# saiprasadbarke/robustmvd

Measured on AMD Instinct MI355X. Metric: depth-maps/sec at 768x1152x4srcx256planes; warp+aggregate HBM GB/s vs roofline, higher is better.
Workload: dtype f32; 1 GPU; mvsnet (Path B) forward 768x1152, 4 source views, 256 planes, batch 1 per step (BASELINE.json configs[2]); the regulariser's two layers with 32 input channels (conv0, conv4): every fp32 operand as two range-scaled fp16 terms on fp16 MFMA, fp32 accumulation (at least as close to a float64 convolution as the fp32 matrix instruction over 1e-42..1e30: tests/test_hip_f16.py), the other nine layers and ; parallelism=1 independent replica(s), frames round-robin, no collectives

## Files before the change

### robustmvd_amd/csrc/warp_variance_tile.hip

```cpp
#include "mvd_common.h"
#include <type_traits>
#include "warp_variance_common.h"

namespace mvd {

typedef unsigned short u16x2 __attribute__((ext_vector_type(2)));

__device__ __forceinline__ unsigned pk_min_u16(unsigned a, unsigned b) {
    return __builtin_bit_cast(unsigned, __builtin_elementwise_min(__builtin_bit_cast(u16x2, a), __builtin_bit_cast(u16x2, b)));
}
__device__ __forceinline__ unsigned pk_max_u16(unsigned a, unsigned b) {
    return __builtin_bit_cast(unsigned, __builtin_elementwise_max(__builtin_bit_cast(u16x2, a), __builtin_bit_cast(u16x2, b)));
}
template <int K>
__device__ __forceinline__ unsigned row_shr(unsigned v) {
    return (unsigned)__builtin_amdgcn_update_dpp((int)v, (int)v, 0x110 + K, 0xf, 0xf, false);
}

typedef float f32x2 __attribute__((ext_vector_type(2)));
struct Sums { f32x2 a1[2], a2[2]; };
__device__ __forceinline__ void tap_pairs(const u32x4& t, f32x2& lo, f32x2& hi) {
    lo = f32x2{__uint_as_float(t.x), __uint_as_float(t.y)};
    hi = f32x2{__uint_as_float(t.z), __uint_as_float(t.w)};
}
__device__ __forceinline__ void tap_pairs(const u32x2& t, f32x2& lo, f32x2& hi) {
    const f16x2 l = as_h2(t.x), h = as_h2(t.y);
    lo = f32x2{(float)l.x, (float)l.y};
    hi = f32x2{(float)h.x, (float)h.y};
}
template <class TAP>
__device__ __forceinline__ void accumulate_cell_pk(Sums& s, const float4 w, const TAP (&t)[4]) {
    const float wk[4] = {w.x, w.y, w.z, w.w};
    f32x2 lo = {0.0f, 0.0f}, hi = {0.0f, 0.0f};
#pragma unroll
    for (int k = 0; k < 4; ++k) {
        f32x2 tl, th;
        tap_pairs(t[k], tl, th);
        const f32x2 ws = {wk[k], wk[k]};
        lo = __builtin_elementwise_fma(tl, ws, lo);
        hi = __builtin_elementwise_fma(th, ws, hi);
    }
    s.a1[0] += lo; s.a1[1] += hi;
    s.a2[0] = __builtin_elementwise_fma(lo, lo, s.a2[0]);
    s.a2[1] = __builtin_elementwise_fma(hi, hi, s.a2[1]);
}

__device__ __forceinline__ void lds_dma_b128(u32x4 rsrc, unsigned voff, unsigned lds_dst) {
    asm volatile("s_mov_b32 m0, %2\n\ts_nop 0\n\tbuffer_load_dwordx4 %0, %1, 0 offen lds" : : "v"(voff), "s"(rsrc), "s"(lds_dst) : "memory");
}

#ifndef MVD_K3T_KO
#define MVD_K3T_KO 0
#endif

struct UnitRec {
    unsigned boxmin;
    unsigned extent;
    unsigned pitch;
    unsigned npix;
    unsigned base;
    unsigned skip;
    float inv_nc;
    unsigned pad;
};
struct ViewRec {
    float M[12];
    unsigned base_lo, base_hi;
    unsigned pad[2];
};

template <int TW, int WINPIX, bool F16, bool EXACT, int MINW, int SETS>
__global__ void __launch_bounds__(256, MINW) warp_variance_tile_kernel(WarpParams p, int nch) {
    constexpr int P = 8, NPX = 32;
    constexpr unsigned PIXB = F16 ? 64 : 128;
    constexpr unsigned QB = F16 ? 8 : 16;
    constexpr unsigned WINB = WINPIX * PIXB;
    constexpr int PPP = 1024 / PIXB;
    constexpr int LPX = PIXB / 16;
    constexpr int NPIECE = WINPIX / PPP;
    constexpr unsigned TABW0 = 2 * WINB, TABO0 = TABW0 + 2 * 4096, PROBE0 = TABO0 + 2 * 1024, FAIL0 = PROBE0 + 512, VIEW0 = FAIL0 + 128;
    using TAP = typename std::conditional<F16, u32x2, u32x4>::type;
    extern __shared__ __attribute__((aligned(16))) char lds[];

    const int tid = threadIdx.x;
    const int wv = __builtin_amdgcn_readfirstlane(tid >> 6);
    const int h = p.h, w = p.w, D = p.D, V = p.V;
    const unsigned DEP0 = VIEW0 + (unsigned)V * sizeof(ViewRec), UNIT0 = DEP0 + (unsigned)nch * 32;

    const int xcd = blockIdx.x & 7;
    int j = blockIdx.x >> 3;
    const int dchunks = (D + P - 1) / P;
    const int dgroups = (dchunks + nch - 1) / nch;
    const int dg = j % dgroups; j /= dgroups;
    const int tile_in = j % p.tiles_per_xcd;
    const int b = j / p.tiles_per_xcd;
    const int tile = xcd * p.tiles_per_xcd + tile_in;
    if (tile >= p.tiles_x * p.tiles_y) return;
    const int tyi = tile / p.tiles_x;
    const int x0 = (tile - tyi * p.tiles_x) * TW, y0 = tyi * (NPX / TW);
    const int nchunks = (dchunks - dg + dgroups - 1) / dgroups;
    auto chunk_of = [&](int jc) { return dg + jc * dgroups; };

    const int W2 = w + 3;
    const unsigned rowb = (unsigned)W2 * PIXB;
    const unsigned img_bytes = (unsigned)(h + 3) * rowb;

    auto opaque_tid = [&]() { int t = tid; asm volatile("" : "+v"(t)); return t; };
    auto blend_pixel = [&](int t, int& bx, int& by) {
        const int px = t >> 3;
        bx = min(x0 + px % TW, w - 1);
        by = min(y0 + px / TW, h - 1);
    };

    float4 key;
    {
        int bx, by;
        blend_pixel(tid, bx, by);
        const char* kp = reinterpret_cast<const char*>(p.key) + (size_t)b * img_bytes + (unsigned)(by + 1) * rowb +
                         (unsigned)(bx + 1) * PIXB + (unsigned)(tid & 7) * QB;
        if constexpr (F16) {
            const u32x2 kh = *reinterpret_cast<const u32x2*>(kp);
            const f16x2 lo = as_h2(kh.x), hi = as_h2(kh.y);
            key = make_float4((float)lo.x, (float)lo.y, (float)hi.x, (float)hi.y);
        } else {
            key = *reinterpret_cast<const float4*>(kp);
        }
    }
    const float inv_nv = 1.0f / (float)(V + 1);
    const size_t plane_bytes = (size_t)h * w * PIXB;

    auto src_rsrc = [&](int v) {
        return __builtin_amdgcn_make_buffer_rsrc(const_cast<char*>(reinterpret_cast<const char*>(p.src.p[v]) + (size_t)b * img_bytes),
                                                 0, (int)img_bytes, 0x00020000);
    };

    const float sx = __int_as_float(__builtin_amdgcn_readfirstlane(__float_as_int((float)w / (float)(w - 1))));
    const float sy = __int_as_float(__builtin_amdgcn_readfirstlane(__float_as_int((float)h / (float)(h - 1))));
    auto position = [&](const float (&M)[12], float fx, float fy, float depth, float& ix, float& iy) -> float {
        float Z;
        if constexpr (EXACT) {
            const float half_w = (float)(w - 1) / 2.0f, half_h = (float)(h - 1) / 2.0f;
            const float gx = fx * depth, gy = fy * depth;
            const float X = ((M[0] * gx + M[1] * gy) + M[2] * depth) + M[3];
            const float Y = ((M[4] * gx + M[5] * gy) + M[6] * depth) + M[7];
            Z = ((M[8] * gx + M[9] * gy) + M[10] * depth) + M[11];
            ix = unnormalize_coord((X / Z) / half_w - 1.0f, (float)w);
            iy = unnormalize_coord((Y / Z) / half_h - 1.0f, (float)h);
        } else {
            const float ax = fmaf(M[0], fx, fmaf(M[1], fy, M[2]));
            const float ay = fmaf(M[4], fx, fmaf(M[5], fy, M[6]));
            const float az = fmaf(M[8], fx, fmaf(M[9], fy, M[10]));
            const float X = fmaf(ax, depth, M[3]), Y = fmaf(ay, depth, M[7]);
            Z = fmaf(az, depth, M[11]);
            const float rz = __builtin_amdgcn_rcpf(Z);
            ix = fmaf(X * rz, sx, -0.5f);
            iy = fmaf(Y * rz, sy, -0.5f);
        }
        ix = __builtin_amdgcn_fmed3f(ix, -1.0f, (float)w);
        iy = __builtin_amdgcn_fmed3f(iy, -1.0f, (float)h);
        return Z;
    };

    unsigned lds_chunks;
    {
        const int pv = tid >> 3, co = tid & 7;
        const float cfx = (float)((co & 1) ? min(x0 + TW - 1, w - 1) : x0);
        const float cfy = (float)((co & 2) ? min(y0 + NPX / TW - 1, h - 1) : y0);
        float M[12];
        {
            const float* Mg = p.M + ((size_t)min(pv, V - 1) * p.B + b) * 12;
#pragma unroll
            for (int k = 0; k < 12; ++k) M[k] = Mg[k];
        }
        if (co == 0 && pv < V) {
            ViewRec* vr = reinterpret_cast<ViewRec*>(lds + VIEW0) + pv;
#pragma unroll
            for (int k = 0; k < 12; ++k) vr->M[k] = M[k];
            const unsigned long long sb = (unsigned long long)(reinterpret_cast<const char*>(p.src.p[pv]) + (size_t)b * img_bytes);
            vr->base_lo = (unsigned)sb; vr->base_hi = (unsigned)(sb >> 32);
        }
        if (tid < 32) *reinterpret_cast<unsigned*>(lds + FAIL0 + tid * 4) = 0u;
        const float* dg_ = p.depth + (size_t)b * D;
        for (int e = tid; e < nchunks * P; e += 256) *reinterpret_cast<float*>(lds + DEP0 + e * 4) = dg_[min(chunk_of(e / P) * P + e % P, D - 1)];
        __syncthreads();
        for (int jc = 0; jc < nchunks; ++jc) {
            const float depth = *reinterpret_cast<const float*>(lds + DEP0 + (jc * P + ((co & 4) ? P - 1 : 0)) * 4);
            float ix, iy;
            const float Z = position(M, cfx, cfy, depth, ix, iy);
            const unsigned cell = ((unsigned)((int)floorf(iy) + 1) << 16) | (unsigned)((int)floorf(ix) + 1);
            const bool ok = Z > 0.0f;
            unsigned mn = ok ? cell : 0u, mx = ok ? cell : 0xffffffffu;
            mn = pk_min_u16(mn, row_shr<1>(mn)); mx = pk_max_u16(mx, row_shr<1>(mx));
            mn = pk_min_u16(mn, row_shr<2>(mn)); mx = pk_max_u16(mx, row_shr<2>(mx));
            mn = pk_min_u16(mn, row_shr<4>(mn)); mx = pk_max_u16(mx, row_shr<4>(mx));
            const int xmin = max((int)(mn & 0xffffu) - 1, 0), ymin = max((int)(mn >> 16) - 1, 0);
            const int xmax = min((int)(mx & 0xffffu) + 1, w + 1), ymax = min((int)(mx >> 16) + 1, h + 1);
            const int nc = xmax - xmin + 2, nr = ymax - ymin + 2;
            const bool mine = (co == 7) && (pv < V);
            if (mine) {
                UnitRec r;
                r.boxmin = (unsigned)xmin | ((unsigned)ymin << 16);
                r.extent = (unsigned)(xmax - xmin) | ((unsigned)(ymax - ymin) << 16);
                r.pitch = (unsigned)nc * PIXB;
                r.npix = (unsigned)(nc * nr);
                r.base = (unsigned)(ymin * W2 + xmin) * PIXB;
                r.skip = rowb - (unsigned)nc * PIXB;
                r.inv_nc = 1.0f / (float)nc;
                r.pad = 0;
                *(reinterpret_cast<UnitRec*>(lds + UNIT0) + jc * V + pv) = r;
            }
            const bool any_bad = __builtin_amdgcn_ballot_w64(mine && nc * nr > WINPIX) != 0;
            if ((tid & 63) == 0) *reinterpret_cast<unsigned*>(lds + PROBE0 + (jc * 4 + wv) * 4) = any_bad ? 1u : 0u;
        }
        __syncthreads();
        unsigned m = 0;
        for (int jc = 0; jc < nchunks; ++jc) {
            const u32x4 f = *reinterpret_cast<const u32x4*>(lds + PROBE0 + jc * 16);
            if ((f.x | f.y | f.z | f.w) == 0) m |= 1u << jc;
        }
        lds_chunks = (unsigned)__builtin_amdgcn_readfirstlane((int)m);
        if constexpr ((MVD_K3T_KO & 16) != 0) lds_chunks = 0;
    }

    auto locate = [&](int jc, int v, int slot, int wb) {
        if constexpr ((MVD_K3T_KO & 8) != 0) return;
        const int t = opaque_tid(), lpx = t & 31, li = t >> 5;
        const float lfx = (float)min(x0 + lpx % TW, w - 1), lfy = (float)min(y0 + lpx / TW, h - 1);
        const float depth = *reinterpret_cast<const float*>(lds + DEP0 + (jc * P + li) * 4);
        const ViewRec* vr = reinterpret_cast<const ViewRec*>(lds + VIEW0) + v;
        const float4 m0 = *reinterpret_cast<const float4*>(vr->M), m1 = *reinterpret_cast<const float4*>(vr->M + 4),
                     m2 = *reinterpret_cast<const float4*>(vr->M + 8);
        const float M[12] = {m0.x, m0.y, m0.z, m0.w, m1.x, m1.y, m1.z, m1.w, m2.x, m2.y, m2.z, m2.w};
        float ix, iy;
        position(M, lfx, lfy, depth, ix, iy);
        const float xf = floorf(ix), yf = floorf(iy);
        const float wx = ix - xf, wy = iy - yf;
        const float ux = 1.0f - wx, uy = 1.0f - wy;
        *reinterpret_cast<float4*>(lds + TABW0 + slot * 4096 + t * 16) = make_float4(ux * uy, wx * uy, ux * wy, wx * wy);
        unsigned* const ent = reinterpret_cast<unsigned*>(lds + TABO0 + slot * 1024 + (lpx * P + li) * 4);
        const int cx = (int)xf + 1, cy = (int)yf + 1;
        if (wb < 0) {
            *ent = (unsigned)(cy * W2 + cx) * PIXB;
        } else {
            const u32x4 rec = *reinterpret_cast<const u32x4*>(lds + UNIT0 + (jc * V + v) * sizeof(UnitRec));
            const unsigned dx = (unsigned)cx - (rec.x & 0xffffu), dy = (unsigned)cy - (rec.x >> 16);
            *ent = (unsigned)wb * WINB + dy * rec.z + dx * PIXB;
            const bool outside = dx > (rec.y & 0xffffu) || dy > (rec.y >> 16);
            if (__builtin_amdgcn_ballot_w64(outside) != 0) {
                if ((t & 63) == 0) *reinterpret_cast<unsigned*>(lds + FAIL0 + jc * 4) = 1u;
            }
        }
    };

    auto copy_window = [&](int jc, int v, int wb) {
        if constexpr ((MVD_K3T_KO & 1) != 0) return;
        const char* rp = lds + UNIT0 + (jc * V + v) * sizeof(UnitRec);
        const u32x4 ra = *reinterpret_cast<const u32x4*>(rp), rb = *reinterpret_cast<const u32x4*>(rp + 16);
        const u32x2 sb = *reinterpret_cast<const u32x2*>(lds + VIEW0 + v * sizeof(ViewRec) + 48);
        const u32x4 rsrc = {(unsigned)__builtin_amdgcn_readfirstlane((int)sb.x), (unsigned)__builtin_amdgcn_readfirstlane((int)sb.y) & 0xffffu,
                            img_bytes, 0x00020000u};
        const int npix = __builtin_amdgcn_readfirstlane((int)ra.w);
        const int ln = opaque_tid() & 63;
        const float inv_nc = __uint_as_float(rb.z);
        const unsigned base = rb.x + (unsigned)(ln % LPX) * 16u + (unsigned)(ln / LPX) * PIXB;
        const float nf0 = (float)(ln / LPX) + 0.5f;
#pragma unroll
        for (int k = 0; k < (NPIECE + 3) / 4; ++k) {
            const int piece = wv + 4 * k;
            if (piece * PPP < npix) {
                const int r = (int)((nf0 + (float)(piece * PPP)) * inv_nc);
                lds_dma_b128(rsrc, base + (unsigned)(piece * 1024) + (unsigned)r * rb.y, (unsigned)(wb * WINB + piece * 1024));
            }
        }
    };

    auto blend = [&](Sums (&sm)[P], int jc, int v, int slot, auto lds_tag) {
        constexpr bool LDSTAPS = decltype(lds_tag)::value;
        const int t = opaque_tid();
        const unsigned q_b = (unsigned)(t & 7) * QB;
        const char* tw = lds + TABW0 + slot * 4096 + (t >> 3) * 16;
        const char* to = lds + TABO0 + slot * 1024 + (t >> 3) * 32;
        const u32x4 oa = *reinterpret_cast<const u32x4*>(to), ob = *reinterpret_cast<const u32x4*>(to + 16);
        const unsigned ofs[P] = {oa.x, oa.y, oa.z, oa.w, ob.x, ob.y, ob.z, ob.w};
        unsigned pitch = 0;
        __amdgpu_buffer_rsrc_t rsrc;
        if constexpr (LDSTAPS) pitch = *reinterpret_cast<const unsigned*>(lds + UNIT0 + (jc * V + v) * sizeof(UnitRec) + 8);
        else rsrc = src_rsrc(v);
        auto weights = [&](int i) { return *reinterpret_cast<const float4*>(tw + i * (NPX * 16)); };
        auto taps = [&](int i, TAP (&f)[4]) {
            const unsigned o = ofs[i] + q_b;
            if constexpr ((MVD_K3T_KO & 2) != 0) {
                if constexpr (F16) { f[0] = u32x2{o, o + 1}; f[1] = u32x2{o + 2, o + 3}; f[2] = u32x2{o + pitch, o + 5}; f[3] = u32x2{o + 6, o + 7}; }
                else { f[0] = u32x4{o, o + 1, o + 2, o + 3}; f[1] = u32x4{o + 4, o + 5, o + 6, o + 7};
                       f[2] = u32x4{o + pitch, o + 9, o + 10, o + 11}; f[3] = u32x4{o + 12, o + 13, o + 14, o + 15}; }
            } else if constexpr (LDSTAPS) {
                f[0] = *reinterpret_cast<const TAP*>(lds + o);
                f[1] = *reinterpret_cast<const TAP*>(lds + o + PIXB);
                f[2] = *reinterpret_cast<const TAP*>(lds + o + pitch);
                f[3] = *reinterpret_cast<const TAP*>(lds + o + pitch + PIXB);
            } else if constexpr (F16) {
                f[0] = load_b64(rsrc, o, 0); f[1] = load_b64(rsrc, o + PIXB, 0);
                f[2] = load_b64(rsrc, o, rowb); f[3] = load_b64(rsrc, o + PIXB, rowb);
            } else {
                f[0] = __builtin_amdgcn_raw_buffer_load_b128(rsrc, o, 0, 0);
                f[1] = __builtin_amdgcn_raw_buffer_load_b128(rsrc, o + PIXB, 0, 0);
                f[2] = __builtin_amdgcn_raw_buffer_load_b128(rsrc, o, rowb, 0);
                f[3] = __builtin_amdgcn_raw_buffer_load_b128(rsrc, o + PIXB, rowb, 0);
            }
        };
        auto next = [&](int i, float4& wq, TAP (&f)[4], Sums& done) {
            wq = weights(i);
            unsigned oi = ofs[i];
            asm volatile("" : "+v"(done.a1[0]), "+v"(done.a1[1]), "+v"(done.a2[0]), "+v"(done.a2[1]), "+v"(oi));
            if (__builtin_amdgcn_ballot_w64(oi != ofs[i - SETS]) != 0) {
                const unsigned o = oi + q_b;
                if constexpr ((MVD_K3T_KO & 2) != 0) { taps(i, f); }
                else if constexpr (LDSTAPS) {
                    f[0] = *reinterpret_cast<const TAP*>(lds + o);
                    f[1] = *reinterpret_cast<const TAP*>(lds + o + PIXB);
                    f[2] = *reinterpret_cast<const TAP*>(lds + o + pitch);
                    f[3] = *reinterpret_cast<const TAP*>(lds + o + pitch + PIXB);
                } else if constexpr (F16) {
                    f[0] = load_b64(rsrc, o, 0); f[1] = load_b64(rsrc, o + PIXB, 0);
                    f[2] = load_b64(rsrc, o, rowb); f[3] = load_b64(rsrc, o + PIXB, rowb);
                } else {
                    f[0] = __builtin_amdgcn_raw_buffer_load_b128(rsrc, o, 0, 0);
                    f[1] = __builtin_amdgcn_raw_buffer_load_b128(rsrc, o + PIXB, 0, 0);
                    f[2] = __builtin_amdgcn_raw_buffer_load_b128(rsrc, o, rowb, 0);
                    f[3] = __builtin_amdgcn_raw_buffer_load_b128(rsrc, o + PIXB, rowb, 0);
                }
            }
        };
        if constexpr (SETS == 2) {
            float4 wA = weights(0), wB = weights(1);
            TAP fA[4], fB[4];
            taps(0, fA);
            taps(1, fB);
            __builtin_amdgcn_sched_barrier(0);
#pragma unroll
            for (int i = 0; i < P; i += 2) {
                accumulate_cell_pk(sm[i], wA, fA);
                __builtin_amdgcn_sched_barrier(0);
                if (i + 2 < P) next(i + 2, wA, fA, sm[i]);
                __builtin_amdgcn_sched_barrier(0);
                accumulate_cell_pk(sm[i + 1], wB, fB);
                __builtin_amdgcn_sched_barrier(0);
                if (i + 3 < P) next(i + 3, wB, fB, sm[i + 1]);
                __builtin_amdgcn_sched_barrier(0);
            }
        } else {
            float4 wA = weights(0);
            TAP fA[4];
            taps(0, fA);
            __builtin_amdgcn_sched_barrier(0);
#pragma unroll
            for (int i = 0; i < P; ++i) {
                accumulate_cell_pk(sm[i], wA, fA);
                __builtin_amdgcn_sched_barrier(0);
                if (i + 1 < P) next(i + 1, wA, fA, sm[i]);
                __builtin_amdgcn_sched_barrier(0);
            }
        }
    };

    auto reset_sums = [&](Sums (&sm)[P]) {
        const f32x2 klo = {key.x, key.y}, khi = {key.z, key.w};
#pragma unroll
        for (int i = 0; i < P; ++i) { sm[i].a1[0] = klo; sm[i].a1[1] = khi; sm[i].a2[0] = klo * klo; sm[i].a2[1] = khi * khi; }
    };

    float amax = 0.f;
    const bool want_absmax = p.absmax != nullptr;
    auto store_chunk = [&](const Sums (&sm)[P], int c, bool drop) {
        int bx, by;
        const int t = opaque_tid();
        blend_pixel(t, bx, by);
        const unsigned out_off = ((unsigned)by * (unsigned)w + (unsigned)bx) * PIXB + (unsigned)(t & 7) * QB;
        const unsigned long long plane0 = (unsigned long long)(reinterpret_cast<char*>(p.out) + ((size_t)b * D + (size_t)c * P) * plane_bytes);
        const int nvalid = drop ? 0 : min(P, D - c * P);
#pragma unroll
        for (int i = 0; i < P; ++i) {
            const float mx = sm[i].a1[0].x * inv_nv, my = sm[i].a1[0].y * inv_nv, mz = sm[i].a1[1].x * inv_nv, mw = sm[i].a1[1].y * inv_nv;
            const float4 r = make_float4(fmaf(sm[i].a2[0].x, inv_nv, -mx * mx), fmaf(sm[i].a2[0].y, inv_nv, -my * my),
                                         fmaf(sm[i].a2[1].x, inv_nv, -mz * mz), fmaf(sm[i].a2[1].y, inv_nv, -mw * mw));
            const unsigned long long pb = plane0 + (i < nvalid ? (unsigned long long)i * plane_bytes : 0ull);
            const __amdgpu_buffer_rsrc_t orsrc = __builtin_amdgcn_make_buffer_rsrc(reinterpret_cast<char*>(pb), 0, i < nvalid ? (int)plane_bytes : 0, 0x00020000);
            if constexpr ((MVD_K3T_KO & 4) != 0) { if (r.x != 123.456f) continue; }
            if (want_absmax && i < nvalid) {
                const float qm = fmaxf(fmaxf(fabsf(r.x), fabsf(r.y)), fmaxf(fabsf(r.z), fabsf(r.w)));
                const bool fin = fabsf(r.x) + fabsf(r.y) + fabsf(r.z) + fabsf(r.w) <= 3.402823466e38f;
                amax = fin ? fmaxf(amax, qm) : amax;
            }
            if constexpr (F16) {
                const f16x2 lo = {(_Float16)r.x, (_Float16)r.y}, hi = {(_Float16)r.z, (_Float16)r.w};
                store_b64(u32x2{as_u32(lo), as_u32(hi)}, orsrc, out_off);
            } else {
                __builtin_amdgcn_raw_buffer_store_b128(u32x4{__float_as_uint(r.x), __float_as_uint(r.y), __float_as_uint(r.z), __float_as_uint(r.w)},
                                                       orsrc, out_off, 0, 0);
            }
        }
    };

#define MVD_UNIT_BARRIER(NST) asm volatile("s_waitcnt vmcnt(" #NST ") lgkmcnt(0)\n\ts_barrier" ::: "memory")
    auto first_chunk = [](unsigned mask) { return mask ? (int)__builtin_ctz(mask) : -1; };
    auto advance = [&](unsigned mask, int& jc, int& v) {
        if (++v < V) return;
        v = 0;
        const unsigned rest = jc >= 31 ? 0u : (mask >> (jc + 1));
        jc = rest ? jc + 1 + (int)__builtin_ctz(rest) : -1;
    };
    std::integral_constant<bool, true> yes;
    std::integral_constant<bool, false> no;

    if (lds_chunks) {
        const unsigned mask = lds_chunks;
        int jb = first_chunk(mask);
        copy_window(jb, 0, 0);
        locate(jb, 0, 0, 0);
        MVD_UNIT_BARRIER(0);
        int slot = 0;
        while (jb >= 0) {
            const unsigned rest = jb >= 31 ? 0u : (mask >> (jb + 1));
            const int jn = rest ? jb + 1 + (int)__builtin_ctz(rest) : -1;
            Sums sm[P];
            reset_sums(sm);
            for (int v = 0; v + 1 < V; ++v) {
                copy_window(jb, v + 1, slot ^ 1);
                blend(sm, jb, v, slot, yes);
                locate(jb, v + 1, slot ^ 1, slot ^ 1);
                MVD_UNIT_BARRIER(0);
                slot ^= 1;
            }
            if (jn >= 0) copy_window(jn, 0, slot ^ 1);
            blend(sm, jb, V - 1, slot, yes);
            {
                const bool drop = __builtin_amdgcn_readfirstlane((int)*reinterpret_cast<const unsigned*>(lds + FAIL0 + jb * 4)) != 0;
                store_chunk(sm, chunk_of(jb), drop);
            }
            if (jn >= 0) locate(jn, 0, slot ^ 1, slot ^ 1);
            MVD_UNIT_BARRIER(8);
            slot ^= 1;
            jb = jn;
        }
    }

    unsigned failed = 0;
    for (int jc = 0; jc < nchunks; ++jc)
        if (*reinterpret_cast<const unsigned*>(lds + FAIL0 + jc * 4) != 0) failed |= 1u << jc;
    failed = (unsigned)__builtin_amdgcn_readfirstlane((int)failed);
    const unsigned all = nchunks >= 32 ? 0xffffffffu : ((1u << nchunks) - 1u);
    const unsigned gmask = (all & ~lds_chunks) | failed;
    if (gmask) {
        int jl = first_chunk(gmask), vl = 0;
        locate(jl, vl, 0, -1); advance(gmask, jl, vl);
        int jb = first_chunk(gmask), vb = 0, slot = 0;
        Sums sm[P];
        reset_sums(sm);
        while (jb >= 0) {
            MVD_UNIT_BARRIER(8);
            if (jl >= 0) { locate(jl, vl, slot ^ 1, -1); advance(gmask, jl, vl); }
            blend(sm, jb, vb, slot, no);
            if (vb + 1 == V) {
                store_chunk(sm, chunk_of(jb), false);
                reset_sums(sm);
            }
            slot ^= 1;
            advance(gmask, jb, vb);
        }
    }
#undef MVD_UNIT_BARRIER
    if (want_absmax) {
        unsigned m = __float_as_uint(amax);
        m = max(m, row_shr<1>(m)); m = max(m, row_shr<2>(m)); m = max(m, row_shr<4>(m)); m = max(m, row_shr<8>(m));
        m = max(m, (unsigned)__builtin_amdgcn_update_dpp((int)m, (int)m, 0x142, 0xa, 0xf, false));
        m = max(m, (unsigned)__builtin_amdgcn_update_dpp((int)m, (int)m, 0x143, 0xc, 0xf, false));
        unsigned* wm = reinterpret_cast<unsigned*>(lds + PROBE0);
        __syncthreads();
        if ((tid & 63) == 63) wm[wv] = m;
        __syncthreads();
        if (tid == 0) raise_absmax(p.absmax, __uint_as_float(max(max(wm[0], wm[1]), max(wm[2], wm[3]))));
    }
}

static size_t tile_lds_bytes(int win, bool f16, int V, int nch) {
    return 2 * (size_t)win * (f16 ? 64 : 128) + 2 * 4096 + 2 * 1024 + 512 + 128 + (size_t)V * sizeof(ViewRec) + (size_t)nch * 32 +
           (size_t)nch * V * sizeof(UnitRec);
}

template <int TW, int WINPIX, bool F16, bool EXACT, int MINW, int SETS>
static int launch_tile_variant(const WarpParams& p, const dim3& grid, hipStream_t st, int nch) {
    const size_t lds = tile_lds_bytes(WINPIX, F16, p.V, nch);
    auto* fn = warp_variance_tile_kernel<TW, WINPIX, F16, EXACT, MINW, SETS>;
    if (lds > 48 * 1024) {
        if (hipFuncSetAttribute(reinterpret_cast<const void*>(fn), hipFuncAttributeMaxDynamicSharedMemorySize, (int)lds) != hipSuccess)
            return launch_status("warp_variance_tile: hipFuncSetAttribute");
    }
    hipLaunchKernelGGL(fn, grid, dim3(256), lds, st, p, nch);
    return MVD_OK;
}

bool warp_tile_supported(const WarpParams& p, bool f16) {
    return p.h + 3 < 65536 && p.w + 3 < 65536 && (long long)p.h * p.w * (f16 ? 64 : 128) < 0x7fffffffLL && p.V <= 32;
}

int launch_warp_tile(const WarpParams& p0, hipStream_t st, int tw, int win, int nch, int sets, bool f16, bool exact) {
    WarpParams p = p0;
    const int th = 32 / tw;
    p.tiles_x = (p.w + tw - 1) / tw;
    p.tiles_y = (p.h + th - 1) / th;
    const long long tiles = (long long)p.tiles_x * p.tiles_y;
    p.tiles_per_xcd = (int)((tiles + 7) / 8);
    const int dchunks = (p.D + 7) / 8;
    nch = nch < 1 ? 1 : (nch > 32 ? 32 : nch);
    const size_t budget = (size_t)160 * 1024 / (sets == 1 ? 4 : 3);
    while (nch > 1 && tile_lds_bytes(win, f16, p.V, nch) > budget) --nch;
    const int dgroups = (dchunks + nch - 1) / nch;
    const long long nblk = 8LL * p.tiles_per_xcd * dgroups * p.B;
    if (nblk > 0x7fffffffLL) {
        set_error("warp_variance: %lld workgroups exceed the grid limit", nblk);
        return MVD_ERR_INVALID_ARG;
    }
    const dim3 grid((unsigned)nblk);
    int rc = MVD_ERR_INVALID_ARG;
    timing_begin(st);
#define MVD_T(TW_, WIN_, MW_, SETS_)                                                                                   \
    if (tw == TW_ && win == WIN_ && sets == SETS_) {                                                                  \
        rc = f16 ? (exact ? launch_tile_variant<TW_, WIN_, true, true, MW_, SETS_>(p, grid, st, nch)                  \
                          : launch_tile_variant<TW_, WIN_, true, false, MW_, SETS_>(p, grid, st, nch))                \
                 : (exact ? launch_tile_variant<TW_, WIN_, false, true, MW_, SETS_>(p, grid, st, nch)                 \
                          : launch_tile_variant<TW_, WIN_, false, false, MW_, SETS_>(p, grid, st, nch));              \
    }
    MVD_T(8, 104, 4, 1) MVD_T(8, 128, 4, 1)
#ifdef MVD_EXPERIMENTS
    MVD_T(8, 128, 3, 2) MVD_T(8, 96, 4, 1) MVD_T(16, 128, 3, 2) MVD_T(16, 104, 4, 1) MVD_T(16, 96, 4, 1) MVD_T(32, 128, 3, 2) MVD_T(32, 104, 4, 1)
#endif
#undef MVD_T
    timing_end(st);
    if (rc == MVD_ERR_INVALID_ARG) {
        set_error("warp_variance: tile variant tw=%d win=%d sets=%d is not compiled", tw, win, sets);
        return rc;
    }
    if (rc) return rc;
    return launch_status("warp_variance_tile");
}

}
```

Measured before the change: 321.3 depth-maps/sec.

## Trim per-unit ALU work in warp-variance tile kernel inner loops

Several micro-optimisations land in the warp-variance tile kernel. The float reciprocal row division in copy_window becomes a 16-bit magic-multiply integer division. The key-seeded accumulator init is folded into the first view's blend, and the view loop is restructured so copy/locate/blend interleave uniformly. Pixel coordinates and the output offset are hoisted out of locate and store_chunk, the ballot in locate becomes a plain per-lane store, and the variance/absmax math is packed (v_max3). The aim is fewer VALU instructions and registers per unit of work, at the risk of subtle indexing bugs in the UnitRec layout change.

```diff
diff --git a/robustmvd_amd/csrc/warp_variance_tile.hip b/robustmvd_amd/csrc/warp_variance_tile.hip
--- a/robustmvd_amd/csrc/warp_variance_tile.hip
+++ b/robustmvd_amd/csrc/warp_variance_tile.hip
@@ -28,8 +28,8 @@
     lo = f32x2{(float)l.x, (float)l.y};
     hi = f32x2{(float)h.x, (float)h.y};
 }
-template <class TAP>
-__device__ __forceinline__ void accumulate_cell_pk(Sums& s, const float4 w, const TAP (&t)[4]) {
+template <bool FIRST, class TAP>
+__device__ __forceinline__ void accumulate_cell_pk(Sums& s, const float4 w, const TAP (&t)[4], const f32x2 (&key)[4]) {
     const float wk[4] = {w.x, w.y, w.z, w.w};
     f32x2 lo = {0.0f, 0.0f}, hi = {0.0f, 0.0f};
 #pragma unroll
@@ -40,9 +40,15 @@
         lo = __builtin_elementwise_fma(tl, ws, lo);
         hi = __builtin_elementwise_fma(th, ws, hi);
     }
-    s.a1[0] += lo; s.a1[1] += hi;
-    s.a2[0] = __builtin_elementwise_fma(lo, lo, s.a2[0]);
-    s.a2[1] = __builtin_elementwise_fma(hi, hi, s.a2[1]);
+    if constexpr (FIRST) {
+        s.a1[0] = key[0] + lo; s.a1[1] = key[1] + hi;
+        s.a2[0] = __builtin_elementwise_fma(lo, lo, key[2]);
+        s.a2[1] = __builtin_elementwise_fma(hi, hi, key[3]);
+    } else {
+        s.a1[0] += lo; s.a1[1] += hi;
+        s.a2[0] = __builtin_elementwise_fma(lo, lo, s.a2[0]);
+        s.a2[1] = __builtin_elementwise_fma(hi, hi, s.a2[1]);
+    }
 }
 
 __device__ __forceinline__ void lds_dma_b128(u32x4 rsrc, unsigned voff, unsigned lds_dst) {
@@ -54,14 +60,13 @@
 #endif
 
 struct UnitRec {
-    unsigned boxmin;
+    int lox, loy;
     unsigned extent;
     unsigned pitch;
     unsigned npix;
     unsigned base;
     unsigned skip;
-    float inv_nc;
-    unsigned pad;
+    unsigned row_magic;
 };
 struct ViewRec {
     float M[12];
@@ -78,6 +83,7 @@
     constexpr int PPP = 1024 / PIXB;
     constexpr int LPX = PIXB / 16;
     constexpr int NPIECE = WINPIX / PPP;
+    static_assert(WINPIX * WINPIX < 65536, "row_magic: window too large for the 16-bit reciprocal");
     constexpr unsigned TABW0 = 2 * WINB, TABO0 = TABW0 + 2 * 4096, PROBE0 = TABO0 + 2 * 1024, FAIL0 = PROBE0 + 512, VIEW0 = FAIL0 + 128;
     using TAP = typename std::conditional<F16, u32x2, u32x4>::type;
     extern __shared__ __attribute__((aligned(16))) char lds[];
@@ -112,10 +118,13 @@
         by = min(y0 + px / TW, h - 1);
     };
 
+    unsigned lxy = (unsigned)min(x0 + (tid & 31) % TW, w - 1) | ((unsigned)min(y0 + (tid & 31) / TW, h - 1) << 16);
+    unsigned out_off;
     float4 key;
     {
         int bx, by;
         blend_pixel(tid, bx, by);
+        out_off = ((unsigned)by * (unsigned)w + (unsigned)bx) * PIXB + (unsigned)(tid & 7) * QB;
         const char* kp = reinterpret_cast<const char*>(p.key) + (size_t)b * img_bytes + (unsigned)(by + 1) * rowb +
                          (unsigned)(bx + 1) * PIXB + (unsigned)(tid & 7) * QB;
         if constexpr (F16) {
@@ -126,6 +135,9 @@
             key = *reinterpret_cast<const float4*>(kp);
         }
     }
+    asm volatile("" : "+v"(lxy), "+v"(out_off));
+    const f32x2 keyp[4] = {f32x2{key.x, key.y}, f32x2{key.z, key.w}, f32x2{key.x, key.y} * f32x2{key.x, key.y},
+                           f32x2{key.z, key.w} * f32x2{key.z, key.w}};
     const float inv_nv = 1.0f / (float)(V + 1);
     const size_t plane_bytes = (size_t)h * w * PIXB;
 
@@ -199,14 +211,13 @@
             const bool mine = (co == 7) && (pv < V);
             if (mine) {
                 UnitRec r;
-                r.boxmin = (unsigned)xmin | ((unsigned)ymin << 16);
+                r.lox = xmin - 1; r.loy = ymin - 1;
                 r.extent = (unsigned)(xmax - xmin) | ((unsigned)(ymax - ymin) << 16);
                 r.pitch = (unsigned)nc * PIXB;
                 r.npix = (unsigned)(nc * nr);
                 r.base = (unsigned)(ymin * W2 + xmin) * PIXB;
                 r.skip = rowb - (unsigned)nc * PIXB;
-                r.inv_nc = 1.0f / (float)nc;
-                r.pad = 0;
+                r.row_magic = (65536u + (unsigned)nc - 1u) / (unsigned)nc;
                 *(reinterpret_cast<UnitRec*>(lds + UNIT0) + jc * V + pv) = r;
             }
             const bool any_bad = __builtin_amdgcn_ballot_w64(mine && nc * nr > WINPIX) != 0;
@@ -225,7 +236,7 @@
     auto locate = [&](int jc, int v, int slot, int wb) {
         if constexpr ((MVD_K3T_KO & 8) != 0) return;
         const int t = opaque_tid(), lpx = t & 31, li = t >> 5;
-        const float lfx = (float)min(x0 + lpx % TW, w - 1), lfy = (float)min(y0 + lpx / TW, h - 1);
+        const float lfx = (float)(lxy & 0xffffu), lfy = (float)(lxy >> 16);
         const float depth = *reinterpret_cast<const float*>(lds + DEP0 + (jc * P + li) * 4);
         const ViewRec* vr = reinterpret_cast<const ViewRec*>(lds + VIEW0) + v;
         const float4 m0 = *reinterpret_cast<const float4*>(vr->M), m1 = *reinterpret_cast<const float4*>(vr->M + 4),
@@ -238,44 +249,43 @@
         const float ux = 1.0f - wx, uy = 1.0f - wy;
         *reinterpret_cast<float4*>(lds + TABW0 + slot * 4096 + t * 16) = make_float4(ux * uy, wx * uy, ux * wy, wx * wy);
         unsigned* const ent = reinterpret_cast<unsigned*>(lds + TABO0 + slot * 1024 + (lpx * P + li) * 4);
-        const int cx = (int)xf + 1, cy = (int)yf + 1;
         if (wb < 0) {
+            const int cx = (int)xf + 1, cy = (int)yf + 1;
             *ent = (unsigned)(cy * W2 + cx) * PIXB;
         } else {
             const u32x4 rec = *reinterpret_cast<const u32x4*>(lds + UNIT0 + (jc * V + v) * sizeof(UnitRec));
-            const unsigned dx = (unsigned)cx - (rec.x & 0xffffu), dy = (unsigned)cy - (rec.x >> 16);
-            *ent = (unsigned)wb * WINB + dy * rec.z + dx * PIXB;
-            const bool outside = dx > (rec.y & 0xffffu) || dy > (rec.y >> 16);
-            if (__builtin_amdgcn_ballot_w64(outside) != 0) {
-                if ((t & 63) == 0) *reinterpret_cast<unsigned*>(lds + FAIL0 + jc * 4) = 1u;
-            }
+            const unsigned dx = (unsigned)((int)xf - (int)rec.x), dy = (unsigned)((int)yf - (int)rec.y);
+            *ent = __umul24(dy, rec.w) + (dx * PIXB + (unsigned)wb * WINB);
+            const bool outside = dx > (rec.z & 0xffffu) || dy > (rec.z >> 16);
+            if (outside) *reinterpret_cast<unsigned*>(lds + FAIL0 + jc * 4) = 1u;
         }
     };
 
     auto copy_window = [&](int jc, int v, int wb) {
         if constexpr ((MVD_K3T_KO & 1) != 0) return;
         const char* rp = lds + UNIT0 + (jc * V + v) * sizeof(UnitRec);
-        const u32x4 ra = *reinterpret_cast<const u32x4*>(rp), rb = *reinterpret_cast<const u32x4*>(rp + 16);
+        const u32x4 rb = *reinterpret_cast<const u32x4*>(rp + 16);
         const u32x2 sb = *reinterpret_cast<const u32x2*>(lds + VIEW0 + v * sizeof(ViewRec) + 48);
         const u32x4 rsrc = {(unsigned)__builtin_amdgcn_readfirstlane((int)sb.x), (unsigned)__builtin_amdgcn_readfirstlane((int)sb.y) & 0xffffu,
                             img_bytes, 0x00020000u};
-        const int npix = __builtin_amdgcn_readfirstlane((int)ra.w);
+        const int npix = __builtin_amdgcn_readfirstlane((int)rb.x);
+        const unsigned magic = (unsigned)__builtin_amdgcn_readfirstlane((int)rb.w);
         const int ln = opaque_tid() & 63;
-        const float inv_nc = __uint_as_float(rb.z);
-        const unsigned base = rb.x + (unsigned)(ln % LPX) * 16u + (unsigned)(ln / LPX) * PIXB;
-        const float nf0 = (float)(ln / LPX) + 0.5f;
+        const unsigned lane_base = rb.y + (unsigned)ln * 16u + (unsigned)(wv * 1024);
+        const unsigned q0 = __umul24((unsigned)(ln / LPX) + (unsigned)(wv * PPP), magic);
 #pragma unroll
         for (int k = 0; k < (NPIECE + 3) / 4; ++k) {
             const int piece = wv + 4 * k;
             if (piece * PPP < npix) {
-                const int r = (int)((nf0 + (float)(piece * PPP)) * inv_nc);
-                lds_dma_b128(rsrc, base + (unsigned)(piece * 1024) + (unsigned)r * rb.y, (unsigned)(wb * WINB + piece * 1024));
-            }
-        }
-    };
-
-    auto blend = [&](Sums (&sm)[P], int jc, int v, int slot, auto lds_tag) {
+                const unsigned r = (q0 + (unsigned)(4 * k * PPP) * magic) >> 16;
+                lds_dma_b128(rsrc, __umul24(r, rb.z) + (unsigned)(4 * k * 1024) + lane_base, (unsigned)(wb * WINB + piece * 1024));
+            }
+        }
+    };
+
+    auto blend = [&](Sums (&sm)[P], int jc, int v, int slot, auto lds_tag, auto first_tag) {
         constexpr bool LDSTAPS = decltype(lds_tag)::value;
+        constexpr bool FIRST = decltype(first_tag)::value;
         const int t = opaque_tid();
         const unsigned q_b = (unsigned)(t & 7) * QB;
         const char* tw = lds + TABW0 + slot * 4096 + (t >> 3) * 16;
@@ -284,7 +294,7 @@
         const unsigned ofs[P] = {oa.x, oa.y, oa.z, oa.w, ob.x, ob.y, ob.z, ob.w};
         unsigned pitch = 0;
         __amdgpu_buffer_rsrc_t rsrc;
-        if constexpr (LDSTAPS) pitch = *reinterpret_cast<const unsigned*>(lds + UNIT0 + (jc * V + v) * sizeof(UnitRec) + 8);
+        if constexpr (LDSTAPS) pitch = *reinterpret_cast<const unsigned*>(lds + UNIT0 + (jc * V + v) * sizeof(UnitRec) + 12);
         else rsrc = src_rsrc(v);
         auto weights = [&](int i) { return *reinterpret_cast<const float4*>(tw + i * (NPX * 16)); };
         auto taps = [&](int i, TAP (&f)[4]) {
@@ -339,11 +349,11 @@
             __builtin_amdgcn_sched_barrier(0);
 #pragma unroll
             for (int i = 0; i < P; i += 2) {
-                accumulate_cell_pk(sm[i], wA, fA);
+                accumulate_cell_pk<FIRST>(sm[i], wA, fA, keyp);
                 __builtin_amdgcn_sched_barrier(0);
                 if (i + 2 < P) next(i + 2, wA, fA, sm[i]);
                 __builtin_amdgcn_sched_barrier(0);
-                accumulate_cell_pk(sm[i + 1], wB, fB);
+                accumulate_cell_pk<FIRST>(sm[i + 1], wB, fB, keyp);
                 __builtin_amdgcn_sched_barrier(0);
                 if (i + 3 < P) next(i + 3, wB, fB, sm[i + 1]);
                 __builtin_amdgcn_sched_barrier(0);
@@ -355,7 +365,7 @@
             __builtin_amdgcn_sched_barrier(0);
 #pragma unroll
             for (int i = 0; i < P; ++i) {
-                accumulate_cell_pk(sm[i], wA, fA);
+                accumulate_cell_pk<FIRST>(sm[i], wA, fA, keyp);
                 __builtin_amdgcn_sched_barrier(0);
                 if (i + 1 < P) next(i + 1, wA, fA, sm[i]);
                 __builtin_amdgcn_sched_barrier(0);
@@ -364,32 +374,30 @@
     };
 
     auto reset_sums = [&](Sums (&sm)[P]) {
-        const f32x2 klo = {key.x, key.y}, khi = {key.z, key.w};
-#pragma unroll
-        for (int i = 0; i < P; ++i) { sm[i].a1[0] = klo; sm[i].a1[1] = khi; sm[i].a2[0] = klo * klo; sm[i].a2[1] = khi * khi; }
+#pragma unroll
+        for (int i = 0; i < P; ++i) { sm[i].a1[0] = keyp[0]; sm[i].a1[1] = keyp[1]; sm[i].a2[0] = keyp[2]; sm[i].a2[1] = keyp[3]; }
     };
 
     float amax = 0.f;
     const bool want_absmax = p.absmax != nullptr;
     auto store_chunk = [&](const Sums (&sm)[P], int c, bool drop) {
-        int bx, by;
-        const int t = opaque_tid();
-        blend_pixel(t, bx, by);
-        const unsigned out_off = ((unsigned)by * (unsigned)w + (unsigned)bx) * PIXB + (unsigned)(t & 7) * QB;
         const unsigned long long plane0 = (unsigned long long)(reinterpret_cast<char*>(p.out) + ((size_t)b * D + (size_t)c * P) * plane_bytes);
         const int nvalid = drop ? 0 : min(P, D - c * P);
 #pragma unroll
         for (int i = 0; i < P; ++i) {
-            const float mx = sm[i].a1[0].x * inv_nv, my = sm[i].a1[0].y * inv_nv, mz = sm[i].a1[1].x * inv_nv, mw = sm[i].a1[1].y * inv_nv;
-            const float4 r = make_float4(fmaf(sm[i].a2[0].x, inv_nv, -mx * mx), fmaf(sm[i].a2[0].y, inv_nv, -my * my),
-                                         fmaf(sm[i].a2[1].x, inv_nv, -mz * mz), fmaf(sm[i].a2[1].y, inv_nv, -mw * mw));
+            const f32x2 inv2 = {inv_nv, inv_nv};
+            const f32x2 mlo = sm[i].a1[0] * inv2, mhi = sm[i].a1[1] * inv2;
+            const f32x2 rlo = __builtin_elementwise_fma(sm[i].a2[0], inv2, -(mlo * mlo)), rhi = __builtin_elementwise_fma(sm[i].a2[1], inv2, -(mhi * mhi));
+            const float4 r = make_float4(rlo.x, rlo.y, rhi.x, rhi.y);
             const unsigned long long pb = plane0 + (i < nvalid ? (unsigned long long)i * plane_bytes : 0ull);
             const __amdgpu_buffer_rsrc_t orsrc = __builtin_amdgcn_make_buffer_rsrc(reinterpret_cast<char*>(pb), 0, i < nvalid ? (int)plane_bytes : 0, 0x00020000);
             if constexpr ((MVD_K3T_KO & 4) != 0) { if (r.x != 123.456f) continue; }
             if (want_absmax && i < nvalid) {
-                const float qm = fmaxf(fmaxf(fabsf(r.x), fabsf(r.y)), fmaxf(fabsf(r.z), fabsf(r.w)));
                 const bool fin = fabsf(r.x) + fabsf(r.y) + fabsf(r.z) + fabsf(r.w) <= 3.402823466e38f;
-                amax = fin ? fmaxf(amax, qm) : amax;
+                float m3, m5;
+                asm("v_max3_f32 %0, |%1|, |%2|, |%3|" : "=v"(m3) : "v"(r.x), "v"(r.y), "v"(r.z));
+                asm("v_max3_f32 %0, %1, %2, |%3|" : "=v"(m5) : "v"(amax), "v"(m3), "v"(r.w));
+                amax = fin ? m5 : amax;
             }
             if constexpr (F16) {
                 const f16x2 lo = {(_Float16)r.x, (_Float16)r.y}, hi = {(_Float16)r.z, (_Float16)r.w};
@@ -422,17 +430,20 @@
         while (jb >= 0) {
             const unsigned rest = jb >= 31 ? 0u : (mask >> (jb + 1));
             const int jn = rest ? jb + 1 + (int)__builtin_ctz(rest) : -1;
+            auto copy_next = [&](int v) {
+                const int cj = v + 1 < V ? jb : jn, cv = v + 1 < V ? v + 1 : 0;
+                if (cj >= 0) copy_window(cj, cv, slot ^ 1);
+            };
             Sums sm[P];
-            reset_sums(sm);
-            for (int v = 0; v + 1 < V; ++v) {
-                copy_window(jb, v + 1, slot ^ 1);
-                blend(sm, jb, v, slot, yes);
-                locate(jb, v + 1, slot ^ 1, slot ^ 1);
+            copy_next(0);
+            blend(sm, jb, 0, slot, yes, yes);
+            for (int v = 1; v < V; ++v) {
+                locate(jb, v, slot ^ 1, slot ^ 1);
                 MVD_UNIT_BARRIER(0);
                 slot ^= 1;
-            }
-            if (jn >= 0) copy_window(jn, 0, slot ^ 1);
-            blend(sm, jb, V - 1, slot, yes);
+                copy_next(v);
+                blend(sm, jb, v, slot, yes, no);
+            }
             {
                 const bool drop = __builtin_amdgcn_readfirstlane((int)*reinterpret_cast<const unsigned*>(lds + FAIL0 + jb * 4)) != 0;
                 store_chunk(sm, chunk_of(jb), drop);
@@ -459,7 +470,7 @@
         while (jb >= 0) {
             MVD_UNIT_BARRIER(8);
             if (jl >= 0) { locate(jl, vl, slot ^ 1, -1); advance(gmask, jl, vl); }
-            blend(sm, jb, vb, slot, no);
+            blend(sm, jb, vb, slot, no, no);
             if (vb + 1 == V) {
                 store_chunk(sm, chunk_of(jb), false);
                 reset_sums(sm);
```

Measured after the change: 320.5 depth-maps/sec (median of 3 runs). About the same (-0.3%).
